# mvenouziou/Boosted_DETR

Measured on AMD Instinct MI355X. Metric: images/sec training step (fwd+matcher+loss+bwd), 640x640 N=100, higher is better.
Workload: dtype f32 (conv/GEMM products as 3 split-f16 [fwd] / split-bf16 [grad] MFMA products, f32 accumulate)

## Files before the change

### boosted_detr_amd/csrc/norm.hip

```cpp
#include "common.h"
#include "p16.h"

namespace {

struct ColGeom { int tx, ty, gx; };
inline ColGeom col_geom(int C) {
    int c4 = C / 4;
    int tx = 1; while (tx < c4 && tx < 64) tx <<= 1;
    ColGeom g; g.tx = tx; g.ty = 256 / tx; g.gx = (c4 + tx - 1) / tx; return g;
}

template <class F>
__global__ __launch_bounds__(256) void colreduce2_kernel(F f, int64_t rows, int C, int tx, int64_t rows_per_chunk,
                                                         float* __restrict__ pa, float* __restrict__ pb) {
    __shared__ f32x4 sa[256], sb[256];
    const int tid = threadIdx.x;
    const int cx = tid % tx, ry = tid / tx, ty = 256 / tx;
    const int c = (blockIdx.x * tx + cx) * 4;
    const int64_t r0 = (int64_t)blockIdx.y * rows_per_chunk;
    const int64_t r1 = min(rows, r0 + rows_per_chunk);
    f32x4 a = {0, 0, 0, 0}, b = {0, 0, 0, 0};
    if (c < C) {
        int64_t r = r0 + ry;
        for (; r + ty < r1; r += 2 * ty) {
            f32x4 qa0, qb0, qa1, qb1;
            f(r, c, qa0, qb0); f(r + ty, c, qa1, qb1);
            a += qa0; b += qb0; a += qa1; b += qb1;
        }
        if (r < r1) { f32x4 qa, qb; f(r, c, qa, qb); a += qa; b += qb; }
    }
    sa[tid] = a; sb[tid] = b;
    __syncthreads();
    for (int s = ty >> 1; s > 0; s >>= 1) {
        if (ry < s) { sa[tid] += sa[tid + s * tx]; sb[tid] += sb[tid + s * tx]; }
        __syncthreads();
    }
    if (ry == 0 && c < C) {
        *reinterpret_cast<f32x4*>(pa + (int64_t)blockIdx.y * C + c) = sa[tid];
        *reinterpret_cast<f32x4*>(pb + (int64_t)blockIdx.y * C + c) = sb[tid];
    }
}

__global__ __launch_bounds__(256) void bn_finalize_kernel(const float* __restrict__ psum, const float* __restrict__ psq, int nparts,
                                                          int64_t rows, int C, float eps, float momentum, int bessel,
                                                          float* mean, float* rstd, float* mmean, float* mvar, int* guard) {
    __shared__ double s1[256], s2[256];
    const int cx = threadIdx.x & 31, py = threadIdx.x >> 5;
    const int c = blockIdx.x * 32 + cx;
    double a = 0, b = 0;
    if (c < C) {
        int p = py;
        for (; p + 3 * 8 < nparts; p += 4 * 8) {
// ... 134 lines not shown
        }
        if (fin.mmean != nullptr && ok) {
            const double vm = (fin.bessel && fin.rows > 1) ? var * ((double)fin.rows / (double)(fin.rows - 1)) : var;
            fin.mmean[c + t] = fin.mmean[c + t] * fin.momentum + (float)m * (1.f - fin.momentum);
            fin.mvar[c + t] = fin.mvar[c + t] * fin.momentum + (float)vm * (1.f - fin.momentum);
        }
    }
}

int wide_reduce_min() {
    static const int n = [] { const char* e = getenv("BDETR_BN_WIDE_REDUCE"); int v = e ? atoi(e) : 0; return v <= 0 ? 0x7fffffff : v; }();
    return n;
}

void sum_partials2(const float* pa, const float* pb, int nparts, int C, float* oa, float* ob, hipStream_t st) {
    if (nparts >= wide_reduce_min() && C % 4 == 0 && (reinterpret_cast<uintptr_t>(pa) | reinterpret_cast<uintptr_t>(pb)) % 16 == 0)
        hipLaunchKernelGGL(reduce_partials2_kernel<false>, dim3(C / 4), dim3(256), 0, st, pa, pb, nparts, C, oa, ob, BnFinalizeArgs{});
    else
        hipLaunchKernelGGL(sum_partials2_kernel, dim3((C + 7) / 8), dim3(256), 0, st, pa, pb, nparts, C, oa, ob);
}

struct StatFn {
    const float* x; int C;
    __device__ __forceinline__ void operator()(int64_t r, int c, f32x4& a, f32x4& b) const {
        f32x4 v = *reinterpret_cast<const f32x4*>(x + r * C + c);
        a = v; b = v * v;
    }
};

__device__ __forceinline__ float bn_affine(float v, float m, float rs, float g, float b) { return __builtin_fmaf(v - m, rs * g, b); }
__device__ __forceinline__ float bn_bwd_dx(float g, float xv, float m, float rs, float gm, float dg, float db, float inv_rows) {
    const float xh = (xv - m) * rs;
    const float t = __builtin_fmaf(-db, inv_rows, g);
    return __builtin_fmaf(-xh, dg * inv_rows, t) * (rs * gm);
}

__device__ __forceinline__ unsigned relu_mask_bits4(const void* mask, int64_t i) {
    const unsigned long long* w = reinterpret_cast<const unsigned long long*>(mask) + (i >> 6) * 4;
    const int b = (int)(i & 63);
    return (unsigned)((w[0] >> b) & 1ull) | ((unsigned)((w[1] >> b) & 1ull) << 1) | ((unsigned)((w[2] >> b) & 1ull) << 2) | ((unsigned)((w[3] >> b) & 1ull) << 3);
}

struct BnBwdFn {
    const float* dout; const float* out; const float* x; const float* mean; const float* rstd; const float* gamma; const float* beta;
    int C; int relu;
    int out_p16 = 0;
    int even_h = 0, even_w = 0;
    int dout_compact = 0;
    __device__ __forceinline__ void operator()(int64_t r, int c, f32x4& a, f32x4& b) const {
        const int64_t rg = r;
        if (even_h > 0) {
            const unsigned w2 = (unsigned)(even_w + 1) >> 1, h2 = (unsigned)(even_h + 1) >> 1;
            const unsigned q = (unsigned)r, j2 = q % w2, t = q / w2, i2 = t % h2, n = t / h2;
            r = ((int64_t)n * even_h + 2 * i2) * even_w + 2 * j2;
        }
        f32x4 g = *reinterpret_cast<const f32x4*>(dout + (dout_compact ? rg : r) * C + c);
        f32x4 xv = *reinterpret_cast<const f32x4*>(x + r * C + c);
        f32x4 m = *reinterpret_cast<const f32x4*>(mean + c);
        f32x4 rs = *reinterpret_cast<const f32x4*>(rstd + c);
        if (relu) {
            if (out != nullptr && out_p16) {
                const unsigned pm = out_p16 == 2 ? relu_mask_bits4(out, (r * C + c) >> 2) : p16_positive4_bf16(out, (r * C + c) >> 2);
#pragma unroll
                for (int e = 0; e < 4; ++e) if (!((pm >> e) & 1u)) g[e] = 0.f;
            } else if (out != nullptr) {
                f32x4 o = *reinterpret_cast<const f32x4*>(out + r * C + c);
#pragma unroll
                for (int e = 0; e < 4; ++e) if (!(o[e] > 0.f)) g[e] = 0.f;
            } else {
                f32x4 gm = *reinterpret_cast<const f32x4*>(gamma + c), bt = *reinterpret_cast<const f32x4*>(beta + c);
#pragma unroll
                for (int e = 0; e < 4; ++e) if (!(bn_affine(xv[e], m[e], rs[e], gm[e], bt[e]) > 0.f)) g[e] = 0.f;
            }
        }
        a = g; b = g * ((xv - m) * rs);
    }
};

__global__ __launch_bounds__(256) void bn_apply_kernel(const float* __restrict__ x, const float* __restrict__ mean, const float* __restrict__ rstd,
                                                       const float* __restrict__ gamma, const float* __restrict__ beta,
                                                       const float* __restrict__ residual, int relu, float* __restrict__ out,
                                                       int64_t n4, int c4n) {
    for (int64_t i = (int64_t)blockIdx.x * blockDim.x + threadIdx.x; i < n4; i += (int64_t)gridDim.x * blockDim.x) {
        const int c = (int)(i % c4n) * 4;
        f32x4 v = reinterpret_cast<const f32x4*>(x)[i];
        f32x4 m = *reinterpret_cast<const f32x4*>(mean + c), rs = *reinterpret_cast<const f32x4*>(rstd + c);
        f32x4 g = *reinterpret_cast<const f32x4*>(gamma + c), b = *reinterpret_cast<const f32x4*>(beta + c);
        f32x4 o;
#pragma unroll
        for (int e = 0; e < 4; ++e) o[e] = bn_affine(v[e], m[e], rs[e], g[e], b[e]);
        if (residual != nullptr) o += reinterpret_cast<const f32x4*>(residual)[i];
        if (relu) {
#pragma unroll
            for (int e = 0; e < 4; ++e) o[e] = fmaxf(o[e], 0.f);
        }
        reinterpret_cast<f32x4*>(out)[i] = o;
    }
}
// ... 61 lines not shown
        f32x4 mx = {-INFINITY, -INFINITY, -INFINITY, -INFINITY};
        unsigned arg = 0;
#pragma unroll
        for (int k = 0; k < 9; ++k) {
            if (!in[k]) continue;
#pragma unroll
            for (int e = 0; e < 4; ++e) {
                const float a = fmaxf(bn_affine(v[k][e], m[e], rs[e], g[e], b[e]), 0.f);
                if (a > mx[e]) { mx[e] = a; arg = (arg & ~(0xFFu << (8 * e))) | ((unsigned)k << (8 * e)); }
            }
        }
        tap[i] = arg;
        if (out32 != nullptr) reinterpret_cast<f32x4*>(out32)[i] = mx;
        if (out_f16 != nullptr) {
            p16_store4<true>(out_f16, i, mx[0], mx[1], mx[2], mx[3]);
            if (overflow_flag != nullptr) {
                const float top = fmaxf(fmaxf(mx[0], mx[1]), fmaxf(mx[2], mx[3]));
                if (!(top < P16_F16_LIMIT)) *overflow_flag = 1;
            }
        }
    }
}

__device__ __forceinline__ f32x4 stem_pixel_grad(const float* __restrict__ dpool, const unsigned* __restrict__ tap, const StemGeom& s, unsigned px, int c,
                                                 const f32x4 yv, const f32x4 m, const f32x4 rs, const f32x4 gm, const f32x4 bt, f32x4& xhat) {
    const int c4n = s.C / 4, c4 = c / 4;
    const int iw = (int)(px % (unsigned)s.W); const unsigned t = px / (unsigned)s.W;
    const int ih = (int)(t % (unsigned)s.H), n = (int)(t / (unsigned)s.H);
    const int ph0 = ih >> 1, pw0 = iw >> 1;
    const bool two_h = (ih & 1) & (int)(ph0 + 1 < s.PH), two_w = (iw & 1) & (int)(pw0 + 1 < s.PW);
    unsigned word[4];
    f32x4 dv[4];
    unsigned mine[4];
#pragma unroll
    for (int k = 0; k < 4; ++k) {
        const int a = k >> 1, b = k & 1;
        const bool real = (a == 0 || two_h) && (b == 0 || two_w);
        const int ph = ph0 + (a & (int)two_h), pw = pw0 + (b & (int)two_w);
        const int64_t o = (((int64_t)n * s.PH + ph) * s.PW + pw) * c4n + c4;
        mine[k] = real ? (unsigned)((ih - (ph * 2 - 1)) * 3 + (iw - (pw * 2 - 1))) : 0xFFu;
        word[k] = tap[o];
        dv[k] = reinterpret_cast<const f32x4*>(dpool)[o];
    }
    f32x4 g = {0.f, 0.f, 0.f, 0.f};
#pragma unroll
    for (int k = 0; k < 4; ++k)
#pragma unroll
        for (int e = 0; e < 4; ++e) if (((word[k] >> (8 * e)) & 0xFFu) == mine[k]) g[e] += dv[k][e];
    xhat = (yv - m) * rs;
#pragma unroll
    for (int e = 0; e < 4; ++e) if (!(bn_affine(yv[e], m[e], rs[e], gm[e], bt[e]) > 0.f)) g[e] = 0.f;
    return g;
}

struct StemBwdFn {
    const float* dpool; const unsigned* tap; const float* y; const float* mean; const float* rstd; const float* gamma; const float* beta; StemGeom s;
    __device__ __forceinline__ void operator()(int64_t r, int c, f32x4& a, f32x4& b) const {
        const f32x4 yv = *reinterpret_cast<const f32x4*>(y + r * s.C + c);
        const f32x4 m = *reinterpret_cast<const f32x4*>(mean + c), rs = *reinterpret_cast<const f32x4*>(rstd + c);
        const f32x4 gm = *reinterpret_cast<const f32x4*>(gamma + c), bt = *reinterpret_cast<const f32x4*>(beta + c);
        f32x4 xh;
        a = stem_pixel_grad(dpool, tap, s, (unsigned)r, c, yv, m, rs, gm, bt, xh);
        b = a * xh;
    }
};

__global__ __launch_bounds__(256) void stem_bwd_apply_kernel(const float* __restrict__ dpool, const unsigned* __restrict__ tap, const float* __restrict__ y,
                                                             const float* __restrict__ mean, const float* __restrict__ rstd, const float* __restrict__ gamma,
                                                             const float* __restrict__ beta, const float* __restrict__ dgamma, const float* __restrict__ dbeta,
                                                             StemGeom s, float* __restrict__ dy, int dy_p16, int64_t n4, float inv_rows) {
    const int c4n = s.C / 4;
    const int64_t stride = (int64_t)gridDim.x * blockDim.x;
    auto one = [&](int64_t i, int c, const f32x4 m, const f32x4 rs, const f32x4 gm, const f32x4 bt, const f32x4 dg, const f32x4 db) {
        const f32x4 yv = reinterpret_cast<const f32x4*>(y)[i];
        f32x4 xh;
        const f32x4 g = stem_pixel_grad(dpool, tap, s, (unsigned)(i / c4n), c, yv, m, rs, gm, bt, xh);
        f32x4 r;
#pragma unroll
        for (int e = 0; e < 4; ++e) r[e] = bn_bwd_dx(g[e], yv[e], m[e], rs[e], gm[e], dg[e], db[e], inv_rows);
        if (dy_p16) p16_store4<false>(dy, i, r[0], r[1], r[2], r[3]);
        else reinterpret_cast<f32x4*>(dy)[i] = r;
    };
    int64_t i = (int64_t)blockIdx.x * blockDim.x + threadIdx.x;
    if (stride % c4n == 0) {
        const int c = (int)(i % c4n) * 4;
// ... 332 lines not shown
    if (row >= rows) return;
    float pv[NPER], dv[NPER];
    float dot = 0.f;
#pragma unroll
    for (int k = 0; k < NPER; ++k) {
        const int c = lane + 64 * k;
        pv[k] = c < cols ? p[row * cols + c] : 0.f;
        dv[k] = c < cols ? dp[row * cols + c] : 0.f;
        dot += pv[k] * dv[k];
    }
    dot = wave_sum(dot);
#pragma unroll
    for (int k = 0; k < NPER; ++k) { const int c = lane + 64 * k; if (c < cols) ds[row * cols + c] = scale * pv[k] * (dv[k] - dot); }
}

int64_t chunks_for_width(int gx) { int64_t c = 2048 / (gx > 0 ? gx : 1); return c < 32 ? 32 : (c > 512 ? 512 : c); }

int64_t chunk_rows_for(int64_t rows, int64_t maxchunks, int64_t minrows) {
    int64_t rpc = cdiv64(rows, maxchunks);
    if (rpc < minrows) rpc = minrows;
    return rpc;
}

}

extern "C" int bdetr_bn_bwd_chunks(int64_t rows) { return (int)cdiv64(rows, chunk_rows_for(rows, 512, 64)); }
extern "C" int bdetr_ln_bwd_chunks(int64_t rows) { return (int)cdiv64(rows, chunk_rows_for(rows, 512, 16)); }

constexpr int BN_FOLD = 64;
extern "C" int bdetr_bn_stats_fold_rows(void) { return BN_FOLD; }

extern "C" int bdetr_bn_stats(const float* x, int64_t rows, int C, const float* part_sum, const float* part_sq,
                              int nparts, float eps, float momentum, int bessel,
                              float* mean, float* rstd, float* moving_mean, float* moving_var, float* fold_ws, int* guard_flag, void* stream) {
    BDETR_CHECK_ARG(mean && rstd && rows > 0 && C > 0, "bdetr_bn_stats: bad arguments");
    BDETR_CHECK_ARG(part_sum != nullptr && part_sq != nullptr && nparts > 0,
                    "bdetr_bn_stats: partial sums required (use bdetr_colstats to produce them from x)");
    (void)x;
    hipStream_t st = (hipStream_t)stream;
    if (nparts >= wide_reduce_min() && C % 4 == 0 && (reinterpret_cast<uintptr_t>(part_sum) | reinterpret_cast<uintptr_t>(part_sq)) % 16 == 0) {
        (void)fold_ws;
        hipLaunchKernelGGL(reduce_partials2_kernel<true>, dim3(C / 4), dim3(256), 0, st, part_sum, part_sq, nparts, C, (float*)nullptr, (float*)nullptr,
                           BnFinalizeArgs{rows, eps, momentum, bessel, mean, rstd, moving_mean, moving_var, guard_flag});
        return bdetr_launch_status("bn_finalize");
    }
    if (nparts > 4 * BN_FOLD && fold_ws != nullptr) {
// ... 24 lines not shown
}

extern "C" int bdetr_bn_apply(const float* x, const float* mean, const float* rstd, const float* gamma,
                              const float* beta, const float* residual, int relu, float* out,
                              int64_t rows, int C, void* stream) {
    BDETR_CHECK_ARG(x && mean && rstd && gamma && beta && out && rows > 0 && C > 0 && C % 4 == 0, "bdetr_bn_apply: bad arguments (C %% 4 == 0 required)");
    int64_t n4 = rows * C / 4;
    hipLaunchKernelGGL(bn_apply_kernel, dim3(ew_grid(n4, 256, 2)), dim3(256), 0, (hipStream_t)stream, x, mean, rstd, gamma, beta, residual, relu, out, n4, C / 4);
    return bdetr_launch_status("bn_apply");
}

extern "C" int bdetr_bn_bwd(const float* dout, const float* out, const float* x, const float* mean,
                            const float* rstd, const float* gamma, const float* beta, int relu, int frozen,
                            float* dx, float* dgamma, float* dbeta, float* dresidual,
                            float* ws, int64_t rows, int C, void* stream) {
    BDETR_CHECK_ARG(dout && x && mean && rstd && gamma && dx && dgamma && dbeta && ws && rows > 0 && C > 0 && C % 4 == 0,
                    "bdetr_bn_bwd: bad arguments (C %% 4 == 0 required)");
    BDETR_CHECK_ARG(!relu || out || beta, "bdetr_bn_bwd: relu needs the forward output, or beta to recompute the mask from x");
    hipStream_t st = (hipStream_t)stream;
    ColGeom g = col_geom(C);
    int64_t rpc = chunk_rows_for(rows, chunks_for_width(g.gx), 64);
    int nch = (int)cdiv64(rows, rpc);
    float* pa = ws; float* pb = ws + (int64_t)nch * C;
    BnBwdFn f{dout, out, x, mean, rstd, gamma, beta, C, relu};
    hipLaunchKernelGGL((colreduce2_kernel<BnBwdFn>), dim3(g.gx, nch), dim3(256), 0, st, f, rows, C, g.tx, rpc, pa, pb);
    sum_partials2(pa, pb, nch, C, dbeta, dgamma, st);
    int64_t n4 = rows * C / 4;
    hipLaunchKernelGGL(bn_bwd_apply_kernel, dim3(ew_grid(n4, 256, 2)), dim3(256), 0, st, dout, out, x, mean, rstd, gamma, beta, dgamma, dbeta,
                       relu, frozen, dx, dresidual, n4, C / 4, 1.0f / (float)rows);
    return bdetr_launch_status("bn_bwd");
}

extern "C" int bdetr_stem_pool_fwd(const float* y, const float* mean, const float* rstd, const float* gamma, const float* beta,
                                   int N, int H, int W, int C, float* out32, void* out_f16, uint8_t* tap, int* overflow_flag, void* stream) {
    BDETR_CHECK_ARG(y && mean && rstd && gamma && beta && tap && (out32 || out_f16) && N > 0 && H > 0 && W > 0 && C > 0 && C % 8 == 0,
                    "bdetr_stem_pool_fwd: bad arguments (C %% 8 == 0 required)");
    BDETR_CHECK_ARG((int64_t)N * H * W < (int64_t)1 << 31, "bdetr_stem_pool_fwd: more than 2^31 pixels");
    const StemGeom s{N, H, W, C, (H + 2 - 3) / 2 + 1, (W + 2 - 3) / 2 + 1};
    const int64_t n4 = (int64_t)N * s.PH * s.PW * (C / 4);
    hipLaunchKernelGGL(stem_pool_fwd_kernel, dim3(ew_grid(n4, 256, 1)), dim3(256), 0, (hipStream_t)stream, y, mean, rstd, gamma, beta, s, out32, out_f16,
                       reinterpret_cast<unsigned*>(tap), overflow_flag);
    return bdetr_launch_status("stem_pool_fwd");
}

constexpr int STEM_BWD_CHUNKS = 2048;
extern "C" int bdetr_stem_pool_bwd_chunks(int64_t rows) { return (int)cdiv64(rows, chunk_rows_for(rows, STEM_BWD_CHUNKS, 64)); }

extern "C" int bdetr_stem_pool_bwd(const float* dpool, const uint8_t* tap, const float* y, const float* mean, const float* rstd, const float* gamma,
// ... 83 lines not shown
    return bdetr_launch_status("relu_mask_apply");
}

static int bn_bwd_p16_impl(const float* dout, const void* out, int out_p16, const float* x, const float* mean,
                           const float* rstd, const float* gamma, const float* beta, int relu, int frozen,
                           float* dx32, void* dx_bf16, float* dgamma, float* dbeta, float* dresidual,
                           float* ws, const float* pre_g, const float* pre_gx, int pre_n, int64_t rows, int C, int even_h, int even_w, void* stream,
                           int dout_compact = 0) {
    BDETR_CHECK_ARG(!dout_compact || (even_h > 0 && even_h % 2 == 0 && even_w % 2 == 0 && pre_g == nullptr && dresidual == nullptr),
                    "bdetr_bn_bwd_p16_even_pixels: a compact dout needs an even map, the even-pixel reduction and no residual-gradient output");
    BDETR_CHECK_ARG(!dout_compact || rows * C / 4 < ((int64_t)1 << 32), "bdetr_bn_bwd_p16_even_pixels: compact dout: more than 2^32 float4s");
    BDETR_CHECK_ARG(dout && x && mean && rstd && gamma && dx_bf16 && dgamma && dbeta && (ws || pre_g) && rows > 0 && C > 0 && C % 8 == 0,
                    "bdetr_bn_bwd_p16: bad arguments (C %% 8 == 0 required)");
    BDETR_CHECK_ARG((pre_g == nullptr) == (pre_gx == nullptr) && (pre_g == nullptr || pre_n > 0), "bdetr_bn_bwd_p16: pre_g / pre_gx / pre_n inconsistent");
    BDETR_CHECK_ARG(!relu || out || beta, "bdetr_bn_bwd_p16: relu needs the forward output, or beta to recompute the mask from x");
    hipStream_t st = (hipStream_t)stream;
    ColGeom g = col_geom(C);
    int64_t rpc = chunk_rows_for(rows, chunks_for_width(g.gx), 64);
    int nch = (int)cdiv64(rows, rpc);
    float* pa = ws; float* pb = ws + (int64_t)nch * C;
    if (pre_g != nullptr) {
        sum_partials2(pre_g, pre_gx, pre_n, C, dbeta, dgamma, st);
    } else {
        BnBwdFn f{dout, reinterpret_cast<const float*>(out), x, mean, rstd, gamma, beta, C, relu, out_p16, even_h, even_w, dout_compact};
        int64_t red_rows = rows;
        if (even_h > 0) {
            red_rows = rows / ((int64_t)even_h * even_w) * ((even_h + 1) / 2) * ((even_w + 1) / 2);
            rpc = chunk_rows_for(red_rows, chunks_for_width(g.gx), 64);
            nch = (int)cdiv64(red_rows, rpc);
            pb = ws + (int64_t)nch * C;
        }
        hipLaunchKernelGGL((colreduce2_kernel<BnBwdFn>), dim3(g.gx, nch), dim3(256), 0, st, f, red_rows, C, g.tx, rpc, pa, pb);
        sum_partials2(pa, pb, nch, C, dbeta, dgamma, st);
    }
    const int64_t n4 = rows * C / 4;
    hipLaunchKernelGGL(bn_bwd_apply_p16_kernel, dim3(channel_aligned_grid(n4, C)), dim3(256), 0, st, dout, out, out_p16, x, mean, rstd, gamma, beta, dgamma, dbeta,
                       relu, frozen, dx32, dx_bf16, dresidual, n4, C / 4, 1.0f / (float)rows, dout_compact ? even_h : 0, dout_compact ? even_w : 0);
    return bdetr_launch_status("bn_bwd_p16");
}

extern "C" int bdetr_bn_bwd_p16(const float* dout, const void* out, int out_p16, const float* x, const float* mean,
                                const float* rstd, const float* gamma, const float* beta, int relu, int frozen,
                                float* dx32, void* dx_bf16, float* dgamma, float* dbeta, float* dresidual,
                                float* ws, const float* pre_g, const float* pre_gx, int pre_n, int64_t rows, int C, void* stream) {
    return bn_bwd_p16_impl(dout, out, out_p16, x, mean, rstd, gamma, beta, relu, frozen, dx32, dx_bf16, dgamma, dbeta, dresidual, ws, pre_g, pre_gx, pre_n,
                           rows, C, 0, 0, stream);
}

extern "C" int bdetr_bn_bwd_p16_even_pixels(const float* dout, const void* out, int out_p16, const float* x, const float* mean,
                                            const float* rstd, const float* gamma, const float* beta, int relu, int frozen,
                                            float* dx32, void* dx_bf16, float* dgamma, float* dbeta, float* dresidual,
                                            float* ws, int N, int H, int W, int C, int dout_compact, void* stream) {
    BDETR_CHECK_ARG(N > 0 && H > 0 && W > 0 && ws && (int64_t)N * H * W < (int64_t)1 << 31, "bdetr_bn_bwd_p16_even_pixels: bad geometry");
    return bn_bwd_p16_impl(dout, out, out_p16, x, mean, rstd, gamma, beta, relu, frozen, dx32, dx_bf16, dgamma, dbeta, dresidual, ws, nullptr, nullptr, 0,
                           (int64_t)N * H * W, C, H, W, stream, dout_compact);
// ... 61 lines not shown
```

### boosted_detr_amd/csrc/p16.h

```cpp
#pragma once
#include "common.h"

typedef unsigned int p16_u32x4 __attribute__((ext_vector_type(4)));
typedef __bf16 p16_bf16x2 __attribute__((ext_vector_type(2)));
typedef _Float16 p16_f16x2 __attribute__((ext_vector_type(2)));
typedef float p16_f32x2 __attribute__((ext_vector_type(2)));

constexpr float P16_W_SCALE = 256.f;
constexpr float P16_F16_LIMIT = 65504.f;

__device__ __forceinline__ void p16_split2_bf16(float x0, float x1, unsigned& hi, unsigned& lo) {
    p16_f32x2 v; v[0] = x0; v[1] = x1;
    hi = __builtin_bit_cast(unsigned, __builtin_convertvector(v, p16_bf16x2));
    p16_f32x2 r;
    r[0] = x0 - __builtin_bit_cast(float, hi << 16);
    r[1] = x1 - __builtin_bit_cast(float, hi & 0xFFFF0000u);
    lo = __builtin_bit_cast(unsigned, __builtin_convertvector(r, p16_bf16x2));
}
__device__ __forceinline__ void p16_split2_f16(float x0, float x1, unsigned& hi, unsigned& lo) {
    p16_f32x2 v; v[0] = x0; v[1] = x1;
    const p16_f16x2 h = __builtin_convertvector(v, p16_f16x2);
    hi = __builtin_bit_cast(unsigned, h);
    const p16_f32x2 r = v - __builtin_convertvector(h, p16_f32x2);
    lo = __builtin_bit_cast(unsigned, __builtin_convertvector(r, p16_f16x2));
// ... 43 lines not shown
    return (unsigned)__builtin_amdgcn_mov_dpp((int)v, 0xB1, 0xF, 0xF, false);
}
template <bool F16>
__device__ __forceinline__ void p16_store4(void* base, int64_t f4_index, float v0, float v1, float v2, float v3) {
    unsigned h01, l01, h23, l23;
    if (F16) { p16_split2_f16(v0, v1, h01, l01); p16_split2_f16(v2, v3, h23, l23); }
    else     { p16_split2_bf16(v0, v1, h01, l01); p16_split2_bf16(v2, v3, h23, l23); }
    const bool odd = (f4_index & 1) != 0;
    const unsigned ra = p16_swap_pair(odd ? h01 : l01), rb = p16_swap_pair(odd ? h23 : l23);
    p16_u32x4 w;
    if (odd) { w[0] = ra; w[1] = rb; w[2] = l01; w[3] = l23; }
    else     { w[0] = h01; w[1] = h23; w[2] = ra; w[3] = rb; }
    reinterpret_cast<p16_u32x4*>(base)[f4_index] = w;
}
__device__ __forceinline__ void p16_load4_f16(const void* base, int64_t f4_index, float (&v)[4]) {
    const char* g = reinterpret_cast<const char*>(base) + (f4_index >> 1) * 32 + (f4_index & 1) * 8;
    const unsigned h0 = reinterpret_cast<const unsigned*>(g)[0], h1 = reinterpret_cast<const unsigned*>(g)[1];
    const unsigned l0 = reinterpret_cast<const unsigned*>(g + 16)[0], l1 = reinterpret_cast<const unsigned*>(g + 16)[1];
    const p16_f32x2 a = __builtin_convertvector(__builtin_bit_cast(p16_f16x2, h0), p16_f32x2), b = __builtin_convertvector(__builtin_bit_cast(p16_f16x2, h1), p16_f32x2);
    const p16_f32x2 c = __builtin_convertvector(__builtin_bit_cast(p16_f16x2, l0), p16_f32x2), d = __builtin_convertvector(__builtin_bit_cast(p16_f16x2, l1), p16_f32x2);
    v[0] = a[0] + c[0]; v[1] = a[1] + c[1];
    v[2] = b[0] + d[0]; v[3] = b[1] + d[1];
}
__device__ __forceinline__ unsigned p16_positive4_bf16(const void* base, int64_t f4_index) {
    const char* g = reinterpret_cast<const char*>(base) + (f4_index >> 1) * 32 + (f4_index & 1) * 8;
    const unsigned h0 = reinterpret_cast<const unsigned*>(g)[0], h1 = reinterpret_cast<const unsigned*>(g)[1];
    auto pos = [](unsigned h16) { return (h16 & 0x8000u) == 0u && (h16 & 0x7FFFu) != 0u; };
    return (pos(h0 & 0xFFFFu) ? 1u : 0u) | (pos(h0 >> 16) ? 2u : 0u) | (pos(h1 & 0xFFFFu) ? 4u : 0u) | (pos(h1 >> 16) ? 8u : 0u);
}
```

### boosted_detr_amd/csrc/rowchain.hip

```cpp
#include "gemm_common.h"
#include "p16.h"

namespace {

typedef unsigned int u32x4 __attribute__((ext_vector_type(4)));
typedef unsigned int u32x2 __attribute__((ext_vector_type(2)));
typedef __bf16 rbf16x8 __attribute__((ext_vector_type(8)));
typedef _Float16 rf16x8 __attribute__((ext_vector_type(8)));

constexpr int RD = 256;
constexpr int RBM = 32;
#ifndef BDETR_RC_WAVES
#define BDETR_RC_WAVES 8
#endif
constexpr int RNW = BDETR_RC_WAVES, RNT = 64 * RNW;
constexpr int TPW = 8 / RNW;
static_assert(RNW == 4 || RNW == 8, "the eight feature tiles split over 4 or 8 waves");
constexpr int ROWB = 2 * RD + 16;
constexpr int PLANE = RBM * ROWB;
#ifndef BDETR_RC_PF
#define BDETR_RC_PF 8
#endif
constexpr int PF = BDETR_RC_PF;
constexpr int KSTEPS = RD / 16;
// ... 403 lines not shown
        tile_to_lds<false>(lds, L, d);
        __syncthreads();
        gemm_stage<false>(w1, wo, lds, L, lane, ring, acc);
        tile_from_acc(acc, d);
#pragma unroll
        for (int t = 0; t < TPW; ++t)
#pragma unroll
            for (int q = 0; q < 4; ++q) d[t][q] += dres[t][q];
        __syncthreads();
    }
    ln_bwd(d, s1t, g1t, mean1, rstd1, red[2], part + 4 * RD, part + 5 * RD, L);
    tile_store(a.dresid, L, d);
    apply_keep(d, a.rate, seed1, L);
    tile_store(a.G0, L, d);
    col_reduce_store(d, part + 6 * RD, L);
    tile_to_lds<false>(lds, L, d);
    __syncthreads();
    gemm_stage<false>(wo, wo, lds, L, lane, ring, acc);
    tile_from_acc(acc, d);
    tile_store(a.dctx, L, d);
}

struct RcReduce { const float* partials; int nparts; float* dst[NVEC]; int accumulate[NVEC]; };
__global__ __launch_bounds__(256) void rowchain_reduce_kernel(RcReduce r) {
    const int v = blockIdx.x, c = threadIdx.x;
    float* dst = v == 0 ? r.dst[0] : v == 1 ? r.dst[1] : v == 2 ? r.dst[2] : v == 3 ? r.dst[3] : v == 4 ? r.dst[4] : v == 5 ? r.dst[5] : r.dst[6];
    const int accum = v == 0 ? r.accumulate[0] : v == 1 ? r.accumulate[1] : v == 2 ? r.accumulate[2] : v == 3 ? r.accumulate[3] : v == 4 ? r.accumulate[4] : v == 5 ? r.accumulate[5] : r.accumulate[6];
    if (dst == nullptr) return;
    const float* p = r.partials + (int64_t)v * RD + c;
    float s0 = 0.f, s1 = 0.f, s2 = 0.f, s3 = 0.f;
    int i = 0;
    for (; i + 4 <= r.nparts; i += 4) {
        s0 += p[(int64_t)(i + 0) * NVEC * RD]; s1 += p[(int64_t)(i + 1) * NVEC * RD];
        s2 += p[(int64_t)(i + 2) * NVEC * RD]; s3 += p[(int64_t)(i + 3) * NVEC * RD];
    }
    for (; i < r.nparts; ++i) s0 += p[(int64_t)i * NVEC * RD];
    const float s = (s0 + s1) + (s2 + s3);
    dst[c] = accum ? dst[c] + s : s;
}

__global__ __launch_bounds__(256) void rowchain_pack_kernel(const int64_t* __restrict__ table, int* __restrict__ overflow) {
    const int64_t* row = table + (int64_t)blockIdx.y * 3;
    const float* w = reinterpret_cast<const float*>(row[0]);
    u32x4* fwd = reinterpret_cast<u32x4*>(row[1]);
    u32x4* bwd = reinterpret_cast<u32x4*>(row[2]);
    const int p = blockIdx.x * 256 + threadIdx.x;
    if (p >= 8 * KSTEPS * 64) return;
    const int lane = p & 63, s = (p >> 6) % KSTEPS, T = p / (64 * KSTEPS);
    const int i = 32 * T + (lane & 31), k0 = 16 * s + 8 * (lane >> 5);
    float a[8], b[8];
    const f32x4 lo4 = *reinterpret_cast<const f32x4*>(w + (int64_t)i * RD + k0), hi4 = *reinterpret_cast<const f32x4*>(w + (int64_t)i * RD + k0 + 4);
#pragma unroll
    for (int e = 0; e < 4; ++e) { a[e] = lo4[e] * P16_W_SCALE; a[4 + e] = hi4[e] * P16_W_SCALE; }
#pragma unroll
    for (int e = 0; e < 8; ++e) b[e] = w[(int64_t)(k0 + e) * RD + i];
    if (overflow != nullptr && p16_f16_overflow(a)) *overflow = 1;
    u32x4 h, l;
    const int64_t base = ((int64_t)(T * KSTEPS + s) * 2) * 64 + lane;
    if (fwd != nullptr) {
#pragma unroll
        for (int e = 0; e < 4; ++e) { unsigned hh, ll; p16_split2_f16(a[2 * e], a[2 * e + 1], hh, ll); h[e] = hh; l[e] = ll; }
// ... 39 lines not shown

extern "C" int bdetr_rowchain_bwd(const bdetr_rowchain_bwd_desc* d, void* stream) {
    BDETR_CHECK_ARG(d && d->M > 0 && (d->nstages == 1 || d->nstages == 3), "bdetr_rowchain_bwd: M > 0 and 1 or 3 stages");
    BDETR_CHECK_ARG(d->dout && d->pre1 && d->mean1 && d->rstd1 && d->g1 && d->wt[0] && d->G0 && d->dresid && d->dctx && d->partials, "bdetr_rowchain_bwd: null pointer (stage 1)");
    BDETR_CHECK_ARG(d->nstages == 1 || (d->pre2 && d->mean2 && d->rstd2 && d->g2 && d->h && d->wt[1] && d->wt[2] && d->G1 && d->G2), "bdetr_rowchain_bwd: null pointer (stages 2-3)");
    bdetr_rowchain_bwd_args a;
    a.M = (int)d->M; a.nstages = d->nstages; a.rate = d->rate; a.dout = d->dout;
    a.pre2 = d->pre2; a.mean2 = d->mean2; a.rstd2 = d->rstd2; a.g2 = d->g2; a.h = d->h; a.pre1 = d->pre1; a.mean1 = d->mean1; a.rstd1 = d->rstd1; a.g1 = d->g1;
    for (int k = 0; k < 3; ++k) a.wt[k] = d->wt[k];
    a.G2 = d->G2; a.G1 = d->G1; a.G0 = d->G0; a.dresid = d->dresid; a.dctx = d->dctx; a.partials = d->partials;
    a.seed1 = d->seed1; a.seed2 = d->seed2; a.seed_base = d->seed_base;
    const bool prof = bdgemm::g_prof_on;
    if (prof) bdgemm::prof_begin((hipStream_t)stream, 2.0 * (double)d->M * RD * RD * d->nstages, (int)d->M, RD, RD * d->nstages, 1, RBM, RD * 10 + 7, bdgemm::AR_BF16X3 * 10000 + 6000);
    hipLaunchKernelGGL(rowchain_bwd_kernel, dim3((unsigned)cdiv64(d->M, RBM)), dim3(RNT), 0, (hipStream_t)stream, a);
    if (prof) bdgemm::prof_end((hipStream_t)stream);
    return bdetr_launch_status("rowchain_bwd");
}

extern "C" int bdetr_rowchain_reduce(const float* partials, int nparts, float* const* dst7, const int* accumulate7, void* stream) {
    BDETR_CHECK_ARG(partials && nparts > 0 && dst7 && accumulate7, "bdetr_rowchain_reduce: bad arguments");
    RcReduce r;
    r.partials = partials; r.nparts = nparts;
    for (int v = 0; v < NVEC; ++v) { r.dst[v] = dst7[v]; r.accumulate[v] = accumulate7[v]; }
    hipLaunchKernelGGL(rowchain_reduce_kernel, dim3(NVEC), dim3(256), 0, (hipStream_t)stream, r);
    return bdetr_launch_status("rowchain_reduce");
}
```

Before: 659.6.

## Batch row loads ahead of math in BN-backward column reductions and rowchain reduce

Splits each column-reduction functor into a load phase and a finish phase. The reduction kernel can then issue 4 rows of loads (2 for the stem) before any math, separated by scheduling barriers, to raise memory-level parallelism. BN backward is templated on its relu-mask mode, which removes runtime branching, and per-column constants are hoisted out of the row loop. The rowchain partial reduce now launches more blocks across columns and issues 64 loads in flight. The cost is more register pressure, with a risk of lower occupancy.

```diff
diff --git a/boosted_detr_amd/csrc/norm.hip b/boosted_detr_amd/csrc/norm.hip
--- a/boosted_detr_amd/csrc/norm.hip
+++ b/boosted_detr_amd/csrc/norm.hip
@@ -9,6 +9,11 @@
     int tx = 1; while (tx < c4 && tx < 64) tx <<= 1;
     ColGeom g; g.tx = tx; g.ty = 256 / tx; g.gx = (c4 + tx - 1) / tx; return g;
 }
+
+template <class F> struct ColRowsInFlight { static constexpr int value = 4; };
+
+struct StemBwdFn;
+template <> struct ColRowsInFlight<StemBwdFn> { static constexpr int value = 2; };
 
 template <class F>
 __global__ __launch_bounds__(256) void colreduce2_kernel(F f, int64_t rows, int C, int tx, int64_t rows_per_chunk,
@@ -21,13 +26,29 @@
     const int64_t r1 = min(rows, r0 + rows_per_chunk);
     f32x4 a = {0, 0, 0, 0}, b = {0, 0, 0, 0};
     if (c < C) {
+        constexpr int ROWS = ColRowsInFlight<F>::value;
+        static_assert(ROWS == 2 || ROWS == 4, "the tail below handles up to three leftover rows");
+        const typename F::Cols k = f.cols(c);
         int64_t r = r0 + ry;
-        for (; r + ty < r1; r += 2 * ty) {
+        for (; r + (ROWS - 1) * (int64_t)ty < r1; r += ROWS * (int64_t)ty) {
+            typename F::Row row[ROWS];
+#pragma unroll
+            for (int u = 0; u < ROWS; ++u) f.load(r + u * (int64_t)ty, c, row[u]);
+            __builtin_amdgcn_sched_barrier(0);
+#pragma unroll
+            for (int u = 0; u < ROWS; ++u) { f32x4 qa, qb; f.finish(row[u], k, c, qa, qb); a += qa; b += qb; }
+            __builtin_amdgcn_sched_barrier(0);
+        }
+        if (ROWS > 2 && r + ty < r1) {
+            typename F::Row row0, row1;
+            f.load(r, c, row0); f.load(r + ty, c, row1);
+            __builtin_amdgcn_sched_barrier(0);
             f32x4 qa0, qb0, qa1, qb1;
-            f(r, c, qa0, qb0); f(r + ty, c, qa1, qb1);
+            f.finish(row0, k, c, qa0, qb0); f.finish(row1, k, c, qa1, qb1);
             a += qa0; b += qb0; a += qa1; b += qb1;
-        }
-        if (r < r1) { f32x4 qa, qb; f(r, c, qa, qb); a += qa; b += qb; }
+            r += 2 * (int64_t)ty;
+        }
+        if (r < r1) { typename F::Row row; f32x4 qa, qb; f.load(r, c, row); f.finish(row, k, c, qa, qb); a += qa; b += qb; }
     }
     sa[tid] = a; sb[tid] = b;
     __syncthreads();
@@ -208,10 +229,11 @@
 
 struct StatFn {
     const float* x; int C;
-    __device__ __forceinline__ void operator()(int64_t r, int c, f32x4& a, f32x4& b) const {
-        f32x4 v = *reinterpret_cast<const f32x4*>(x + r * C + c);
-        a = v; b = v * v;
-    }
+    struct Cols {};
+    struct Row { f32x4 v; };
+    __device__ __forceinline__ Cols cols(int) const { return Cols{}; }
+    __device__ __forceinline__ void load(int64_t r, int c, Row& w) const { w.v = *reinterpret_cast<const f32x4*>(x + r * C + c); }
+    __device__ __forceinline__ void finish(const Row& w, const Cols&, int, f32x4& a, f32x4& b) const { a = w.v; b = w.v * w.v; }
 };
 
 __device__ __forceinline__ float bn_affine(float v, float m, float rs, float g, float b) { return __builtin_fmaf(v - m, rs * g, b); }
@@ -221,45 +243,70 @@
     return __builtin_fmaf(-xh, dg * inv_rows, t) * (rs * gm);
 }
 
-__device__ __forceinline__ unsigned relu_mask_bits4(const void* mask, int64_t i) {
+struct ReluMaskWords { unsigned long long w[4]; };
+__device__ __forceinline__ ReluMaskWords relu_mask_words(const void* mask, int64_t i) {
     const unsigned long long* w = reinterpret_cast<const unsigned long long*>(mask) + (i >> 6) * 4;
-    const int b = (int)(i & 63);
-    return (unsigned)((w[0] >> b) & 1ull) | ((unsigned)((w[1] >> b) & 1ull) << 1) | ((unsigned)((w[2] >> b) & 1ull) << 2) | ((unsigned)((w[3] >> b) & 1ull) << 3);
-}
-
-struct BnBwdFn {
+    return ReluMaskWords{{w[0], w[1], w[2], w[3]}};
+}
+__device__ __forceinline__ unsigned relu_mask_bits4(const ReluMaskWords& m, int b) {
+    return (unsigned)((m.w[0] >> b) & 1ull) | ((unsigned)((m.w[1] >> b) & 1ull) << 1) | ((unsigned)((m.w[2] >> b) & 1ull) << 2) | ((unsigned)((m.w[3] >> b) & 1ull) << 3);
+}
+__device__ __forceinline__ unsigned relu_mask_bits4(const void* mask, int64_t i) { return relu_mask_bits4(relu_mask_words(mask, i), (int)(i & 63)); }
+
+struct BnBwdArgs {
     const float* dout; const float* out; const float* x; const float* mean; const float* rstd; const float* gamma; const float* beta;
     int C; int relu;
     int out_p16 = 0;
     int even_h = 0, even_w = 0;
     int dout_compact = 0;
-    __device__ __forceinline__ void operator()(int64_t r, int c, f32x4& a, f32x4& b) const {
+};
+enum BnBwdMask { BNM_NONE = 0, BNM_OUT32 = 1, BNM_OUT_BF16 = 2, BNM_BITS = 3, BNM_RECOMPUTE = 4 };
+inline int bn_bwd_mask_mode(const BnBwdArgs& f) {
+    if (!f.relu) return BNM_NONE;
+    if (f.out != nullptr) return f.out_p16 == 2 ? BNM_BITS : f.out_p16 ? BNM_OUT_BF16 : BNM_OUT32;
+    return BNM_RECOMPUTE;
+}
+template <int MODE>
+struct BnBwdFn : BnBwdArgs {
+    struct Cols { f32x4 m, rs, gm, bt; };
+    struct Row { f32x4 g, xv, o; ReluMaskWords bits; unsigned h0, h1; int bit; };
+    __device__ __forceinline__ Cols cols(int c) const {
+        Cols k;
+        k.m = *reinterpret_cast<const f32x4*>(mean + c); k.rs = *reinterpret_cast<const f32x4*>(rstd + c);
+        k.gm = k.bt = f32x4{0.f, 0.f, 0.f, 0.f};
+        if constexpr (MODE == BNM_RECOMPUTE) { k.gm = *reinterpret_cast<const f32x4*>(gamma + c); k.bt = *reinterpret_cast<const f32x4*>(beta + c); }
+        return k;
+    }
+    __device__ __forceinline__ void load(int64_t r, int c, Row& w) const {
         const int64_t rg = r;
         if (even_h > 0) {
             const unsigned w2 = (unsigned)(even_w + 1) >> 1, h2 = (unsigned)(even_h + 1) >> 1;
             const unsigned q = (unsigned)r, j2 = q % w2, t = q / w2, i2 = t % h2, n = t / h2;
             r = ((int64_t)n * even_h + 2 * i2) * even_w + 2 * j2;
         }
-        f32x4 g = *reinterpret_cast<const f32x4*>(dout + (dout_compact ? rg : r) * C + c);
-        f32x4 xv = *reinterpret_cast<const f32x4*>(x + r * C + c);
-        f32x4 m = *reinterpret_cast<const f32x4*>(mean + c);
-        f32x4 rs = *reinterpret_cast<const f32x4*>(rstd + c);
-        if (relu) {
-            if (out != nullptr && out_p16) {
-                const unsigned pm = out_p16 == 2 ? relu_mask_bits4(out, (r * C + c) >> 2) : p16_positive4_bf16(out, (r * C + c) >> 2);
-#pragma unroll
-                for (int e = 0; e < 4; ++e) if (!((pm >> e) & 1u)) g[e] = 0.f;
-            } else if (out != nullptr) {
-                f32x4 o = *reinterpret_cast<const f32x4*>(out + r * C + c);
-#pragma unroll
-                for (int e = 0; e < 4; ++e) if (!(o[e] > 0.f)) g[e] = 0.f;
-            } else {
-                f32x4 gm = *reinterpret_cast<const f32x4*>(gamma + c), bt = *reinterpret_cast<const f32x4*>(beta + c);
-#pragma unroll
-                for (int e = 0; e < 4; ++e) if (!(bn_affine(xv[e], m[e], rs[e], gm[e], bt[e]) > 0.f)) g[e] = 0.f;
-            }
-        }
-        a = g; b = g * ((xv - m) * rs);
+        w.g = *reinterpret_cast<const f32x4*>(dout + (dout_compact ? rg : r) * C + c);
+        w.xv = *reinterpret_cast<const f32x4*>(x + r * C + c);
+        const int64_t i = (r * C + c) >> 2;
+        if constexpr (MODE == BNM_BITS) { w.bits = relu_mask_words(out, i); w.bit = (int)(i & 63); }
+        else if constexpr (MODE == BNM_OUT_BF16) {
+            const unsigned* h = reinterpret_cast<const unsigned*>(reinterpret_cast<const char*>(out) + (i >> 1) * 32 + (i & 1) * 8);
+            w.h0 = h[0]; w.h1 = h[1];
+        } else if constexpr (MODE == BNM_OUT32) w.o = *reinterpret_cast<const f32x4*>(out + r * C + c);
+    }
+    __device__ __forceinline__ void finish(const Row& w, const Cols& k, int, f32x4& a, f32x4& b) const {
+        f32x4 g = w.g;
+        if constexpr (MODE == BNM_BITS || MODE == BNM_OUT_BF16) {
+            const unsigned pm = MODE == BNM_BITS ? relu_mask_bits4(w.bits, w.bit) : p16_positive4_bf16_words(w.h0, w.h1);
+#pragma unroll
+            for (int e = 0; e < 4; ++e) if (!((pm >> e) & 1u)) g[e] = 0.f;
+        } else if constexpr (MODE == BNM_OUT32) {
+#pragma unroll
+            for (int e = 0; e < 4; ++e) if (!(w.o[e] > 0.f)) g[e] = 0.f;
+        } else if constexpr (MODE == BNM_RECOMPUTE) {
+#pragma unroll
+            for (int e = 0; e < 4; ++e) if (!(bn_affine(w.xv[e], k.m[e], k.rs[e], k.gm[e], k.bt[e]) > 0.f)) g[e] = 0.f;
+        }
+        a = g; b = g * ((w.xv - k.m) * k.rs);
     }
 };
 
@@ -367,45 +414,58 @@
     }
 }
 
-__device__ __forceinline__ f32x4 stem_pixel_grad(const float* __restrict__ dpool, const unsigned* __restrict__ tap, const StemGeom& s, unsigned px, int c,
-                                                 const f32x4 yv, const f32x4 m, const f32x4 rs, const f32x4 gm, const f32x4 bt, f32x4& xhat) {
+struct StemTaps { unsigned word[4]; f32x4 dv[4]; unsigned mine; };
+__device__ __forceinline__ void stem_taps_load(const float* __restrict__ dpool, const unsigned* __restrict__ tap, const StemGeom& s, unsigned px, int c, StemTaps& w) {
     const int c4n = s.C / 4, c4 = c / 4;
     const int iw = (int)(px % (unsigned)s.W); const unsigned t = px / (unsigned)s.W;
     const int ih = (int)(t % (unsigned)s.H), n = (int)(t / (unsigned)s.H);
     const int ph0 = ih >> 1, pw0 = iw >> 1;
     const bool two_h = (ih & 1) & (int)(ph0 + 1 < s.PH), two_w = (iw & 1) & (int)(pw0 + 1 < s.PW);
-    unsigned word[4];
-    f32x4 dv[4];
-    unsigned mine[4];
+    w.mine = 0u;
 #pragma unroll
     for (int k = 0; k < 4; ++k) {
         const int a = k >> 1, b = k & 1;
         const bool real = (a == 0 || two_h) && (b == 0 || two_w);
         const int ph = ph0 + (a & (int)two_h), pw = pw0 + (b & (int)two_w);
         const int64_t o = (((int64_t)n * s.PH + ph) * s.PW + pw) * c4n + c4;
-        mine[k] = real ? (unsigned)((ih - (ph * 2 - 1)) * 3 + (iw - (pw * 2 - 1))) : 0xFFu;
-        word[k] = tap[o];
-        dv[k] = reinterpret_cast<const f32x4*>(dpool)[o];
-    }
+        w.mine |= (real ? (unsigned)((ih - (ph * 2 - 1)) * 3 + (iw - (pw * 2 - 1))) : 0xFFu) << (8 * k);
+        w.word[k] = tap[o];
+        w.dv[k] = reinterpret_cast<const f32x4*>(dpool)[o];
+    }
+}
+__device__ __forceinline__ f32x4 stem_taps_grad(const StemTaps& w, const f32x4 yv, const f32x4 m, const f32x4 rs, const f32x4 gm, const f32x4 bt, f32x4& xhat) {
     f32x4 g = {0.f, 0.f, 0.f, 0.f};
 #pragma unroll
     for (int k = 0; k < 4; ++k)
 #pragma unroll
-        for (int e = 0; e < 4; ++e) if (((word[k] >> (8 * e)) & 0xFFu) == mine[k]) g[e] += dv[k][e];
+        for (int e = 0; e < 4; ++e) if (((w.word[k] >> (8 * e)) & 0xFFu) == ((w.mine >> (8 * k)) & 0xFFu)) g[e] += w.dv[k][e];
     xhat = (yv - m) * rs;
 #pragma unroll
     for (int e = 0; e < 4; ++e) if (!(bn_affine(yv[e], m[e], rs[e], gm[e], bt[e]) > 0.f)) g[e] = 0.f;
     return g;
 }
+__device__ __forceinline__ f32x4 stem_pixel_grad(const float* __restrict__ dpool, const unsigned* __restrict__ tap, const StemGeom& s, unsigned px, int c,
+                                                 const f32x4 yv, const f32x4 m, const f32x4 rs, const f32x4 gm, const f32x4 bt, f32x4& xhat) {
+    StemTaps w;
+    stem_taps_load(dpool, tap, s, px, c, w);
+    return stem_taps_grad(w, yv, m, rs, gm, bt, xhat);
+}
 
 struct StemBwdFn {
     const float* dpool; const unsigned* tap; const float* y; const float* mean; const float* rstd; const float* gamma; const float* beta; StemGeom s;
-    __device__ __forceinline__ void operator()(int64_t r, int c, f32x4& a, f32x4& b) const {
-        const f32x4 yv = *reinterpret_cast<const f32x4*>(y + r * s.C + c);
-        const f32x4 m = *reinterpret_cast<const f32x4*>(mean + c), rs = *reinterpret_cast<const f32x4*>(rstd + c);
-        const f32x4 gm = *reinterpret_cast<const f32x4*>(gamma + c), bt = *reinterpret_cast<const f32x4*>(beta + c);
+    struct Cols { f32x4 m, rs, gm, bt; };
+    struct Row { f32x4 yv; StemTaps taps; };
+    __device__ __forceinline__ Cols cols(int c) const {
+        return Cols{*reinterpret_cast<const f32x4*>(mean + c), *reinterpret_cast<const f32x4*>(rstd + c), *reinterpret_cast<const f32x4*>(gamma + c),
+                    *reinterpret_cast<const f32x4*>(beta + c)};
+    }
+    __device__ __forceinline__ void load(int64_t r, int c, Row& w) const {
+        w.yv = *reinterpret_cast<const f32x4*>(y + r * s.C + c);
+        stem_taps_load(dpool, tap, s, (unsigned)r, c, w.taps);
+    }
+    __device__ __forceinline__ void finish(const Row& w, const Cols& k, int, f32x4& a, f32x4& b) const {
         f32x4 xh;
-        a = stem_pixel_grad(dpool, tap, s, (unsigned)r, c, yv, m, rs, gm, bt, xh);
+        a = stem_taps_grad(w.taps, w.yv, k.m, k.rs, k.gm, k.bt, xh);
         b = a * xh;
     }
 };
@@ -784,6 +844,17 @@
     return rpc;
 }
 
+void launch_bn_bwd_reduce(const BnBwdArgs& f, const ColGeom& g, int nch, int64_t rows, int64_t rpc, float* pa, float* pb, hipStream_t st) {
+    const dim3 grid(g.gx, nch);
+    switch (bn_bwd_mask_mode(f)) {
+    case BNM_NONE:      hipLaunchKernelGGL((colreduce2_kernel<BnBwdFn<BNM_NONE>>), grid, dim3(256), 0, st, BnBwdFn<BNM_NONE>{f}, rows, f.C, g.tx, rpc, pa, pb); break;
+    case BNM_OUT32:     hipLaunchKernelGGL((colreduce2_kernel<BnBwdFn<BNM_OUT32>>), grid, dim3(256), 0, st, BnBwdFn<BNM_OUT32>{f}, rows, f.C, g.tx, rpc, pa, pb); break;
+    case BNM_OUT_BF16:  hipLaunchKernelGGL((colreduce2_kernel<BnBwdFn<BNM_OUT_BF16>>), grid, dim3(256), 0, st, BnBwdFn<BNM_OUT_BF16>{f}, rows, f.C, g.tx, rpc, pa, pb); break;
+    case BNM_BITS:      hipLaunchKernelGGL((colreduce2_kernel<BnBwdFn<BNM_BITS>>), grid, dim3(256), 0, st, BnBwdFn<BNM_BITS>{f}, rows, f.C, g.tx, rpc, pa, pb); break;
+    default:            hipLaunchKernelGGL((colreduce2_kernel<BnBwdFn<BNM_RECOMPUTE>>), grid, dim3(256), 0, st, BnBwdFn<BNM_RECOMPUTE>{f}, rows, f.C, g.tx, rpc, pa, pb); break;
+    }
+}
+
 }
 
 extern "C" int bdetr_bn_bwd_chunks(int64_t rows) { return (int)cdiv64(rows, chunk_rows_for(rows, 512, 64)); }
@@ -854,8 +925,8 @@
     int64_t rpc = chunk_rows_for(rows, chunks_for_width(g.gx), 64);
     int nch = (int)cdiv64(rows, rpc);
     float* pa = ws; float* pb = ws + (int64_t)nch * C;
-    BnBwdFn f{dout, out, x, mean, rstd, gamma, beta, C, relu};
-    hipLaunchKernelGGL((colreduce2_kernel<BnBwdFn>), dim3(g.gx, nch), dim3(256), 0, st, f, rows, C, g.tx, rpc, pa, pb);
+    BnBwdArgs f{dout, out, x, mean, rstd, gamma, beta, C, relu};
+    launch_bn_bwd_reduce(f, g, nch, rows, rpc, pa, pb, st);
     sum_partials2(pa, pb, nch, C, dbeta, dgamma, st);
     int64_t n4 = rows * C / 4;
     hipLaunchKernelGGL(bn_bwd_apply_kernel, dim3(ew_grid(n4, 256, 2)), dim3(256), 0, st, dout, out, x, mean, rstd, gamma, beta, dgamma, dbeta,
@@ -985,7 +1056,7 @@
     if (pre_g != nullptr) {
         sum_partials2(pre_g, pre_gx, pre_n, C, dbeta, dgamma, st);
     } else {
-        BnBwdFn f{dout, reinterpret_cast<const float*>(out), x, mean, rstd, gamma, beta, C, relu, out_p16, even_h, even_w, dout_compact};
+        BnBwdArgs f{dout, reinterpret_cast<const float*>(out), x, mean, rstd, gamma, beta, C, relu, out_p16, even_h, even_w, dout_compact};
         int64_t red_rows = rows;
         if (even_h > 0) {
             red_rows = rows / ((int64_t)even_h * even_w) * ((even_h + 1) / 2) * ((even_w + 1) / 2);
@@ -993,7 +1064,7 @@
             nch = (int)cdiv64(red_rows, rpc);
             pb = ws + (int64_t)nch * C;
         }
-        hipLaunchKernelGGL((colreduce2_kernel<BnBwdFn>), dim3(g.gx, nch), dim3(256), 0, st, f, red_rows, C, g.tx, rpc, pa, pb);
+        launch_bn_bwd_reduce(f, g, nch, red_rows, rpc, pa, pb, st);
         sum_partials2(pa, pb, nch, C, dbeta, dgamma, st);
     }
     const int64_t n4 = rows * C / 4;
diff --git a/boosted_detr_amd/csrc/p16.h b/boosted_detr_amd/csrc/p16.h
--- a/boosted_detr_amd/csrc/p16.h
+++ b/boosted_detr_amd/csrc/p16.h
@@ -89,9 +89,11 @@
     v[0] = a[0] + c[0]; v[1] = a[1] + c[1];
     v[2] = b[0] + d[0]; v[3] = b[1] + d[1];
 }
-__device__ __forceinline__ unsigned p16_positive4_bf16(const void* base, int64_t f4_index) {
-    const char* g = reinterpret_cast<const char*>(base) + (f4_index >> 1) * 32 + (f4_index & 1) * 8;
-    const unsigned h0 = reinterpret_cast<const unsigned*>(g)[0], h1 = reinterpret_cast<const unsigned*>(g)[1];
+__device__ __forceinline__ unsigned p16_positive4_bf16_words(unsigned h0, unsigned h1) {
     auto pos = [](unsigned h16) { return (h16 & 0x8000u) == 0u && (h16 & 0x7FFFu) != 0u; };
     return (pos(h0 & 0xFFFFu) ? 1u : 0u) | (pos(h0 >> 16) ? 2u : 0u) | (pos(h1 & 0xFFFFu) ? 4u : 0u) | (pos(h1 >> 16) ? 8u : 0u);
 }
+__device__ __forceinline__ unsigned p16_positive4_bf16(const void* base, int64_t f4_index) {
+    const char* g = reinterpret_cast<const char*>(base) + (f4_index >> 1) * 32 + (f4_index & 1) * 8;
+    return p16_positive4_bf16_words(reinterpret_cast<const unsigned*>(g)[0], reinterpret_cast<const unsigned*>(g)[1]);
+}
diff --git a/boosted_detr_amd/csrc/rowchain.hip b/boosted_detr_amd/csrc/rowchain.hip
--- a/boosted_detr_amd/csrc/rowchain.hip
+++ b/boosted_detr_amd/csrc/rowchain.hip
@@ -449,21 +449,44 @@
 }
 
 struct RcReduce { const float* partials; int nparts; float* dst[NVEC]; int accumulate[NVEC]; };
-__global__ __launch_bounds__(256) void rowchain_reduce_kernel(RcReduce r) {
-    const int v = blockIdx.x, c = threadIdx.x;
+constexpr int RC_RED_ROWS = 64, RC_RED_COLS = 64;
+__global__ __launch_bounds__(RC_RED_COLS) void rowchain_reduce_kernel(RcReduce r) {
+    const int v = blockIdx.x, c = blockIdx.y * RC_RED_COLS + threadIdx.x;
     float* dst = v == 0 ? r.dst[0] : v == 1 ? r.dst[1] : v == 2 ? r.dst[2] : v == 3 ? r.dst[3] : v == 4 ? r.dst[4] : v == 5 ? r.dst[5] : r.dst[6];
     const int accum = v == 0 ? r.accumulate[0] : v == 1 ? r.accumulate[1] : v == 2 ? r.accumulate[2] : v == 3 ? r.accumulate[3] : v == 4 ? r.accumulate[4] : v == 5 ? r.accumulate[5] : r.accumulate[6];
     if (dst == nullptr) return;
+    const float d0 = accum ? dst[c] : 0.f;
+    constexpr int64_t step = (int64_t)NVEC * RD;
     const float* p = r.partials + (int64_t)v * RD + c;
+    const int n = r.nparts, n4 = n & ~3;
     float s0 = 0.f, s1 = 0.f, s2 = 0.f, s3 = 0.f;
     int i = 0;
-    for (; i + 4 <= r.nparts; i += 4) {
-        s0 += p[(int64_t)(i + 0) * NVEC * RD]; s1 += p[(int64_t)(i + 1) * NVEC * RD];
-        s2 += p[(int64_t)(i + 2) * NVEC * RD]; s3 += p[(int64_t)(i + 3) * NVEC * RD];
-    }
-    for (; i < r.nparts; ++i) s0 += p[(int64_t)i * NVEC * RD];
+    for (; i + RC_RED_ROWS <= n4; i += RC_RED_ROWS) {
+        float x[RC_RED_ROWS];
+#pragma unroll
+        for (int u = 0; u < RC_RED_ROWS; ++u) x[u] = p[(i + u) * step];
+        __builtin_amdgcn_sched_barrier(0);
+#pragma unroll
+        for (int u = 0; u < RC_RED_ROWS; u += 4) { s0 += x[u]; s1 += x[u + 1]; s2 += x[u + 2]; s3 += x[u + 3]; }
+        __builtin_amdgcn_sched_barrier(0);
+    }
+    {
+        float x[RC_RED_ROWS - 4], t[3];
+#pragma unroll
+        for (int u = 0; u < RC_RED_ROWS - 4; ++u) x[u] = p[(i + (u | 3) < n4 ? i + u : 0) * step];
+#pragma unroll
+        for (int k = 0; k < 3; ++k) t[k] = p[(n4 + k < n ? n4 + k : 0) * step];
+        __builtin_amdgcn_sched_barrier(0);
+#pragma unroll
+        for (int u = 0; u < RC_RED_ROWS - 4; u += 4) {
+            const bool ok = i + u + 3 < n4;
+            s0 = ok ? s0 + x[u] : s0; s1 = ok ? s1 + x[u + 1] : s1; s2 = ok ? s2 + x[u + 2] : s2; s3 = ok ? s3 + x[u + 3] : s3;
+        }
+#pragma unroll
+        for (int k = 0; k < 3; ++k) s0 = n4 + k < n ? s0 + t[k] : s0;
+    }
     const float s = (s0 + s1) + (s2 + s3);
-    dst[c] = accum ? dst[c] + s : s;
+    dst[c] = accum ? d0 + s : s;
 }
 
 __global__ __launch_bounds__(256) void rowchain_pack_kernel(const int64_t* __restrict__ table, int* __restrict__ overflow) {
@@ -549,6 +572,6 @@
     RcReduce r;
     r.partials = partials; r.nparts = nparts;
     for (int v = 0; v < NVEC; ++v) { r.dst[v] = dst7[v]; r.accumulate[v] = accumulate7[v]; }
-    hipLaunchKernelGGL(rowchain_reduce_kernel, dim3(NVEC), dim3(256), 0, (hipStream_t)stream, r);
+    hipLaunchKernelGGL(rowchain_reduce_kernel, dim3(NVEC, RD / RC_RED_COLS), dim3(RC_RED_COLS), 0, (hipStream_t)stream, r);
     return bdetr_launch_status("rowchain_reduce");
 }
```

After: 660.7 (median of 4 runs). Within noise of the previous version (+0.2%).
